# biodatageeks/polars-bio

Measured on AMD Instinct MI355X. Metric: overlap-pairs/sec, higher is better.
Workload: dtype int32; 1 GPU; overlap_100M_5M_24contig; probe_rows=100000000, build_rows=5000000, contigs=24, filter_op=Strict, parallelism=single GPU

## Files before the change

polars-bio_amd/csrc/host_index.hip.h:

```cpp
#pragma once

namespace {

int build_tables(ivj_ctx* ctx, ivj_index* ix);
bool cs_geom(int64_t n, int nc, int want_rows, CsGeom& g);
size_t cs_index_bytes(const CsGeom& g);
void cs_index_carve(ivj_index* ix, char* p);

int ensure_hier(ivj_ctx* ctx, ivj_index* ix) {
    if (ix->hier_built || ix->n <= 0) return IVJ_OK;
    const HierShape h = hier_shape(ix->n);
    const int64_t wgs = (((ix->n + 15) & ~(int64_t)15) + HIER_WG_ROWS - 1) / HIER_WG_ROWS;
    LAUNCH(ctx, "hier_low", k_hier_low, (unsigned)wgs, 256, (const int2*)ix->ep, ix->n, ix->hier, h);
    if (h.nlev >= 3) LAUNCH(ctx, "hier_high", k_hier_high, 1, 256, ix->hier, h, wgs);
    HIP_TRY(hipGetLastError());
    ix->hier_built = true;
    return IVJ_OK;
}

int need_tables(ivj_ctx* ctx, ivj_index* ix) {
    if (!ix->has_tables) return fail(IVJ_ESTATE, "this index was built for merge / cluster only (with_end_order & 2): it has no lookup tables");
    if (ix->tables_built) return IVJ_OK;
    return build_tables(ctx, ix);
}
// ... 91 lines not shown
        int bins_per_row = 2;
        if (ctx->env_joint_bins == 1 || ctx->env_joint_bins == 2) bins_per_row = ctx->env_joint_bins;
        LAUNCH(ctx, "contig_meta", k_contig_meta_joint, grid1d(ix->n_contigs, 256), 256, (const int32_t*)ix->seg,
               (const int32_t*)ix->b_start, (const int32_t*)ix->e_end, ix->n_contigs, bins_per_row, ix->cmeta_j);
        HIP_TRY(hipMemsetAsync(jb_s, 0, (size_t)ix->bins_len * 4, ctx->stream));
        HIP_TRY(hipMemsetAsync(jb_e, 0, (size_t)ix->bins_len * 4, ctx->stream));
        LAUNCH(ctx, "bins_mark", k_bins_mark, grid1d(n, 256), 256, (const int32_t*)ix->b_start, (const int32_t*)ix->b_contig, n,
               ix->n_contigs, (const int4*)ix->cmeta_j, jb_s);
        LAUNCH(ctx, "bins_mark", k_bins_mark, grid1d(n, 256), 256, (const int32_t*)ix->e_end, (const int32_t*)ckeys, n,
               ix->n_contigs, (const int4*)ix->cmeta_j, jb_e);
        lb_max_scan(jb_s, 0);
        lb_max_scan(jb_e, 1);
        LAUNCH(ctx, "joint_records", k_joint_records, grid1d(ix->bins_len, 256), 256, (const uint32_t*)jb_s, (const uint32_t*)jb_e,
               ix->bins_len, (const int32_t*)ix->b_start, (const int32_t*)ix->e_end, (const int4*)ix->cmeta_j, ix->n_contigs, ix->crec);
    }
    ix->has_end_order = true;
    return IVJ_OK;
}

int build_end_table(ivj_ctx* ctx, ivj_index* ix) {
    IVJ_TRY(build_end_order(ctx, ix));
    if (ix->has_end_table || ix->n == 0 || ix->n_contigs <= 0) { ix->has_end_table = true; return IVJ_OK; }
    const int64_t n = ix->n;
    const int64_t lb_tiles = (ix->bins_len + LB_TILE - 1) / LB_TILE;
    const size_t zb = align_up((size_t)lb_tiles * 8) + align_up(16);
    IVJ_TRY(arena_reserve(ctx, zb + 4096));
    char* z = arena_take<char>(ctx, zb);
    HIP_TRY(hipMemsetAsync(z, 0, zb, ctx->stream));
    LAUNCH(ctx, "contig_meta", k_contig_meta, grid1d(ix->n_contigs, 256), 256, (const int32_t*)ix->seg,
           (const int32_t*)ix->e_end, ix->n_contigs, ix->cmeta_e);
    HIP_TRY(hipMemsetAsync(ix->bins_e, 0, (size_t)ix->bins_len * 4, ctx->stream));
    LAUNCH(ctx, "bins_mark", k_bins_mark, grid1d(n, 256), 256, (const int32_t*)ix->e_end, (const int32_t*)ix->b_contig, n,
           ix->n_contigs, (const int4*)ix->cmeta_e, ix->bins_e);
    LAUNCH(ctx, "bins_scan", (k_scan_lb_u32<MaxOp, false>), lb_tiles, OS_THREADS, ix->bins_e, ix->bins_len, 0u,
           (uint32_t*)(z + align_up((size_t)lb_tiles * 8)), (unsigned long long*)z);
    LAUNCH(ctx, "bins_records", k_bins_records, grid1d(ix->bins_len, 256), 256, (const uint32_t*)ix->bins_e, ix->bins_len,
           (const int32_t*)ix->e_end, (const int4*)ix->cmeta_e, ix->n_contigs, ix->brec_e);
    HIP_TRY(hipGetLastError());
    ix->has_end_table = true;
    return IVJ_OK;
}

int build_argmax(ivj_ctx* ctx, ivj_index* ix) {
    if (ix->has_argmax) return IVJ_OK;
    const int64_t n = ix->n;
    if (n == 0) { ix->has_argmax = true; return IVJ_OK; }
    LAUNCH(ctx, "pmax_change", k_pmax_change, grid1d(n, 256), 256, (const int2*)ix->ep, (const int32_t*)ix->b_contig, n, (uint32_t*)ix->pargmax);
    IVJ_TRY((lb_scan_u32<MaxOp, false>(ctx, "argmax_scan", (uint32_t*)ix->pargmax, n, 0u)));
    LAUNCH(ctx, "nearest_records", k_nearest_records, grid1d(n + 1, 256), 256, (const int32_t*)ix->b_start, (const int2*)ix->ep,
           (const int32_t*)ix->b_row, (const int32_t*)ix->b_contig, (const int32_t*)ix->pargmax, n, ix->nrec);
    ix->has_argmax = true;
    return IVJ_OK;
}

int build_lines(ivj_ctx* ctx, ivj_index* ix) {
    if (ix->has_lines) return IVJ_OK;
    if (!ix->has_tables) return fail(IVJ_ESTATE, "this index was built for merge / cluster only (with_end_order & 2): it has no lookup tables");
    const size_t need = (size_t)ix->bins_len * 64;
    if (ix->nline_cap < need) {
        if (ix->nline) { (void)hipFree(ix->nline); ix->nline = nullptr; ix->nline_cap = 0; }
        if (ctx->nl_cache && ctx->nl_cache_cap >= need) {
            ix->nline = reinterpret_cast<int4*>(ctx->nl_cache); ix->nline_cap = ctx->nl_cache_cap;
            ctx->nl_cache = nullptr; ctx->nl_cache_cap = 0;
        } else {
            hipError_t e = hipMalloc((void**)&ix->nline, need);
            if (e != hipSuccess) { ix->nline = nullptr; return fail(IVJ_ENOMEM, std::string("hipMalloc(nearest lines): ") + hipGetErrorString(e)); }
            ix->nline_cap = need;
        }
    }
    IVJ_TRY(need_tables(ctx, ix));
    IVJ_TRY(build_argmax(ctx, ix));
    LAUNCH(ctx, "nearest_lines", k_nearest_lines, grid1d(ix->bins_len * 4, 256), 256, (const uint32_t*)ix->bins, (const int4*)ix->cmeta, ix->n_contigs, (const int4*)ix->nrec,
           (const int32_t*)ix->b_start, (const int2*)ix->ep, (const int32_t*)ix->b_row, ix->bins_len, ix->n, ix->nline);
    HIP_TRY(hipGetLastError());
    ix->has_lines = true;
    return IVJ_OK;
}

int build_rec4(ivj_ctx* ctx, ivj_index* ix) {
    if (ix->has_rec4 || ix->n == 0) return IVJ_OK;
    LAUNCH(ctx, "rec4", k_rec4, grid1d(ix->n, 256), 256, (const int32_t*)ix->b_start, (const int2*)ix->ep, (const int32_t*)ix->b_row, ix->n, ix->rec4);
    HIP_TRY(hipGetLastError());
    ix->has_rec4 = true;
    return IVJ_OK;
}

int build_flat(ivj_ctx* ctx, ivj_index* ix) {
    if (ix->has_flat || ix->n == 0 || ix->n_contigs <= 0) return IVJ_OK;
    IVJ_TRY(need_tables(ctx, ix));
    HIP_TRY(hipMemsetAsync(ix->lot, 0, (size_t)ix->bins_len * 4, ctx->stream));
    LAUNCH(ctx, "lot_mark", k_lot_mark, grid1d(ix->n, 256), 256, (const int2*)ix->ep, (const int32_t*)ix->b_contig, ix->n,
           ix->n_contigs, (const int4*)ix->cmeta, ix->lot);
    IVJ_TRY((lb_scan_u32<MaxOp, false>(ctx, "lot_scan", ix->lot, ix->bins_len, 0u)));
    LAUNCH(ctx, "tab2", k_tab2, grid1d(ix->bins_len, 256), 256, (const uint32_t*)ix->bins, (const uint32_t*)ix->lot, ix->bins_len, ix->tab2);
    HIP_TRY(hipGetLastError());
    IVJ_TRY(build_rec4(ctx, ix));
    ix->has_flat = true;
    return IVJ_OK;
}

int index_sort_v2(ivj_ctx* ctx, ivj_index* ix, const ivj_side* build, const ivj_opts* opts) {
    OsSort S;
    IVJ_TRY(arena_reserve(ctx, os_sort_plan(S, build->n, opts->n_contigs) + 4096));
    os_sort_take(ctx, S);
    IVJ_TRY(os_sort_run(ctx, S, build->contig, build->start, build->end, build->row_id));
    LAUNCH(ctx, "ix_final", k_ix_final, S.tiles, OS_THREADS, (const int4*)S.recA, (const int4*)S.recB, S.n, S.nc, S.cbits, S.meta, S.st_fin, ix->b_start, ix->ep, ix->b_row,
           ix->b_contig, ix->seg, ix->flags);
    HIP_TRY(hipGetLastError());
    return IVJ_OK;
}

bool ix3_wanted(const ivj_ctx* ctx, int64_t n, int nc) {
    if (nc + 1 > V3_MAX_KEYS || n <= 0 || n > (int64_t)V3_CAP * V3_BUCKETS) return false;
    if (ctx->env_ix_v3 >= 0) return ctx->env_ix_v3 != 0;
    if (ctx->ix3_fallback_streak >= 2 && (ctx->ix3_builds_since_fallback & 15) != 15) return false;
    return n >= (128ll << 10) && n <= (7ll << 20);
}
struct V3Plan { int64_t chunk, hist_len, hs_tiles; int nchunks; size_t z_meta, z_st, z_hs, z_tick, zero_bytes; };
V3Plan v3_plan(int64_t n) {
    V3Plan p;
    p.chunk = ((n + 255) / 256 + OS_TILE - 1) / OS_TILE * OS_TILE;
    if (p.chunk < OS_TILE) p.chunk = OS_TILE;
    p.nchunks = (int)((n + p.chunk - 1) / p.chunk);
    p.hist_len = (int64_t)V3_BUCKETS * p.nchunks;
    p.hs_tiles = (p.hist_len + LB_TILE - 1) / LB_TILE;
    p.z_meta = align_up(sizeof(V3Meta)); p.z_st = align_up((size_t)V3_BUCKETS * 8); p.z_hs = align_up((size_t)p.hs_tiles * 8); p.z_tick = align_up(16);
    p.zero_bytes = p.z_meta + p.z_st + p.z_hs + p.z_tick;
    return p;
}
int index_sort_v3(ivj_ctx* ctx, ivj_index* ix, const ivj_side* build, const ivj_opts* opts, bool* done) {
    *done = false;
    const int64_t n = build->n;
    const int nc = opts->n_contigs;
    const int64_t tiles = (n + OS_TILE - 1) / OS_TILE;
    const V3Plan VP = v3_plan(n);
    const int64_t chunk = VP.chunk, hist_len = VP.hist_len, hs_tiles = VP.hs_tiles;
    const int nchunks = VP.nchunks;
    const size_t z_meta = VP.z_meta, z_st = VP.z_st, z_hs = VP.z_hs, zero_bytes = VP.zero_bytes;
    OsSort S;
    const size_t v2_bytes = os_sort_plan(S, n, nc);
    const bool own_z = ix->ix3_z == nullptr;
    IVJ_TRY(arena_reserve(ctx, std::max(v2_bytes, (own_z ? zero_bytes : 0) + align_up((size_t)hist_len * 4) + align_up((size_t)n * 16)) + 4096));
    char* z = own_z ? arena_take<char>(ctx, zero_bytes) : ix->ix3_z;
    uint32_t* hist = arena_take<uint32_t>(ctx, (size_t)hist_len);
    int4* recs = arena_take<int4>(ctx, (size_t)n);
    V3Meta* meta = (V3Meta*)z;
    unsigned long long* st_local = (unsigned long long*)(z + z_meta);
    unsigned long long* st_scan = (unsigned long long*)(z + z_meta + z_st);
    uint32_t* tick_scan = (uint32_t*)(z + z_meta + z_st + z_hs);
    if (own_z) HIP_TRY(hipMemsetAsync(z, 0, zero_bytes, ctx->stream));
    const size_t pass_lds = (size_t)v3_pass_lds().total;
    if (!ctx->ix3_attr_set) {
        HIP_TRY(hipFuncSetAttribute(reinterpret_cast<const void*>(&k_v3_scatter), hipFuncAttributeMaxDynamicSharedMemorySize, (int)pass_lds));
        HIP_TRY(hipFuncSetAttribute(reinterpret_cast<const void*>(&k_v3_local<true>), hipFuncAttributeMaxDynamicSharedMemorySize, 160 * 1024 - 256));
        HIP_TRY(hipFuncSetAttribute(reinterpret_cast<const void*>(&k_v3_local<false>), hipFuncAttributeMaxDynamicSharedMemorySize, 160 * 1024 - 256));
        ctx->ix3_attr_set = true;
    }
    const unsigned sgrid = (unsigned)(tiles < 512 ? tiles : 512);
    LAUNCH(ctx, "ix3_stats", k_v3_stats, sgrid, OS_THREADS, build->start, build->end, build->contig, n, nc, meta);
    LAUNCH(ctx, "ix3_hist", k_v3_hist, nchunks, OS_THREADS, build->contig, build->start, n, nc, meta, (int)chunk, nchunks, hist);
    LAUNCH(ctx, "ix_scan", (k_scan_lb_u32<SumOp, true>), hs_tiles, OS_THREADS, hist, hist_len, 0u, tick_scan, st_scan);
    const int ms_max = ctx->env_ix_merge >= 0 ? std::min(ctx->env_ix_merge, V3_MAX_MERGE) : V3_MAX_MERGE;
    const uint32_t hw_seq = ctx->hw ? ++ctx->hw_seq : 0u;
    LAUNCH(ctx, "ix3_check", k_v3_check, 1, OS_THREADS, (const uint32_t*)hist, nchunks, n, ms_max, meta, ctx->hw_dev, hw_seq);
    if (!ctx->hw) HIP_TRY(hipMemcpyAsync(ctx->h_total + 6, &meta->bad, 8, hipMemcpyDeviceToHost, ctx->stream));
    if (!ctx->ix3_event) HIP_TRY(hipEventCreateWithFlags(&ctx->ix3_event, hipEventDisableTiming));
    HIP_TRY(hipEventRecord(ctx->ix3_event, ctx->stream));
    t_begin(ctx, "ix3_pass");
    hipLaunchKernelGGL(k_v3_scatter, dim3((unsigned)nchunks), dim3(OS_THREADS), pass_lds, ctx->stream, build->contig, build->start, build->end, build->row_id,
                       recs, n, nc, meta, (int)chunk, nchunks, (const uint32_t*)hist);
    t_end(ctx);
    HIP_TRY(hipGetLastError());
    HIP_TRY(wait_event(ctx, ctx->ix3_event));
    uint32_t* hv = reinterpret_cast<uint32_t*>(ctx->h_total + 6);
    if (ctx->hw) {
        const volatile uint32_t* w = reinterpret_cast<volatile uint32_t*>(ctx->hw);
        if (w[2] == hw_seq) { hv[0] = w[0]; hv[1] = w[1]; }
        else {
            ++ctx->hw_misses;
            HIP_TRY(hipMemcpyAsync(ctx->h_total + 6, &meta->bad, 8, hipMemcpyDeviceToHost, ctx->stream));
            HIP_TRY(hipStreamSynchronize(ctx->stream));
        }
    }
    const uint32_t max_bucket = hv[1] & 0xffffffu;
    const int ms = (int)(hv[1] >> 24);
    if (hv[0] != 0u || max_bucket > (uint32_t)V3_CAP) { ++ctx->ix3_fallbacks; ++ctx->ix3_fallback_streak; ctx->ix3_builds_since_fallback = 0; return IVJ_OK; }
    ctx->ix3_fallback_streak = 0;
    const int cap = (int)std::max<uint32_t>(1024u, (max_bucket + 1023u) / 1024u * 1024u);
    const int bin_bits = cap <= 1024 ? 10 : (cap <= 2048 ? 11 : V3_MAX_BIN_BITS);
    const bool stage = ctx->env_ix_stage >= 0 ? ctx->env_ix_stage != 0 : cap <= 2048;
    const size_t local_lds = (size_t)v3_local_lds(cap, 1 << bin_bits, stage).total;
    with_bool(stage, [&](auto STAGE) {
        LAUNCH_LDS(ctx, "ix3_local", k_v3_local<STAGE>, V3_BUCKETS >> ms, OS_THREADS, local_lds, (const int4*)recs, (const uint32_t*)hist, nchunks, n, nc, cap, bin_bits, ms,
                   meta, st_local, ix->b_start, ix->ep, ix->b_row, ix->b_contig, ix->seg, ix->flags);
    });
    HIP_TRY(hipGetLastError());
    *done = true;
    return IVJ_OK;
}

int build_tables(ivj_ctx* ctx, ivj_index* ix) {
    const int nc = ix->n_contigs;
    const int64_t n = ix->n;
    if (n > 0 && nc > 0) {
        const int64_t lb_tiles = (ix->bins_len + LB_TILE - 1) / LB_TILE;
        const size_t zb = align_up((size_t)lb_tiles * 8) + align_up(16);
        IVJ_TRY(arena_reserve(ctx, zb + 4096));
        char* z = arena_take<char>(ctx, zb);
        HIP_TRY(hipMemsetAsync(z, 0, zb, ctx->stream));
        HIP_TRY(hipMemsetAsync(ix->bins, 0, (size_t)ix->bins_len * 4, ctx->stream));
        LAUNCH(ctx, "contig_meta", k_contig_meta, grid1d(nc, 256), 256, (const int32_t*)ix->seg, (const int32_t*)ix->b_start, nc, ix->cmeta);
        LAUNCH(ctx, "bins_mark", k_bins_mark, grid1d(n, 256), 256, (const int32_t*)ix->b_start, (const int32_t*)ix->b_contig, n, nc,
               (const int4*)ix->cmeta, ix->bins);
        LAUNCH(ctx, "bins_scan", (k_scan_lb_u32<MaxOp, false>), lb_tiles, OS_THREADS, ix->bins, ix->bins_len, 0u,
               (uint32_t*)(z + align_up((size_t)lb_tiles * 8)), (unsigned long long*)z);
        LAUNCH(ctx, "bins_records", k_bins_records, grid1d(ix->bins_len, 256), 256, (const uint32_t*)ix->bins, ix->bins_len,
               (const int32_t*)ix->b_start, (const int4*)ix->cmeta, nc, ix->brec);
        HIP_TRY(hipGetLastError());
    }
    ix->tables_built = true;
    return IVJ_OK;
}

int index_build(ivj_ctx* ctx, const ivj_side* build, const ivj_opts* opts, int with_end_order, ivj_index** out) {
    if (2 * build->n + 2 * (int64_t)opts->n_contigs + 64 > 0x7fffffffll)
        return fail(IVJ_EINVAL, "build side too large for the int32 direct-address table (2*rows + 2*contigs must be < 2^31)");
    ivj_index* ix = new ivj_index();
    ix->ctx = ctx; ix->device = ctx->device; ix->n = build->n; ix->n_contigs = opts->n_contigs; ix->table_mode = opts->table_mode;
    const int64_t n = build->n;
    const size_t nn = (size_t)(n > 0 ? n : 1);
    auto cleanup = [&](int code) { ivj_index_free(ix); return code; };
    {
        const size_t col = align_up(nn * 4);
        const size_t nc = (size_t)opts->n_contigs;
        ix->bins_len = 2 * (int64_t)nn + 2 * (int64_t)nc + 16;
        const size_t v3z = (n > 0 && ix3_wanted(ctx, n, opts->n_contigs)) ? v3_plan(n).zero_bytes : 0;
        const size_t small = align_up((nc + 2) * 4) + align_up(16) + 3 * align_up((nc + 1) * 32) + v3z;
        const size_t flat_bytes = align_up((nn + 1) * 16) + 3 * align_up((size_t)ix->bins_len * 4);
        const size_t spl_bytes = align_up((size_t)SL_MAX_BUCKETS * 8) + align_up((size_t)SL_TAB_CONTIGS * 16) +
                                 align_up((size_t)(4 * SL_MAX_BUCKETS + 2 * SL_TAB_CONTIGS) * 4);
        ix->cs_ok = n > 0 && cs_geom(n, opts->n_contigs, opts->slice_rows > 0 ? opts->slice_rows : ctx->sl_env_rows, ix->cs_g);
        const size_t cs_bytes = ix->cs_ok ? cs_index_bytes(ix->cs_g) : 0;
        const size_t hier_bytes = align_up(hier_shape((int64_t)nn).values * 4);
        const size_t need = hier_bytes + cs_bytes + spl_bytes + flat_bytes + 6 * col + align_up(nn * 8) + align_up((nn + 1) * 32) + 2 * align_up((size_t)ix->bins_len * 4) +
                            3 * align_up((size_t)ix->bins_len * 16) + small + 256;
        if (ctx->ix_cache && ctx->ix_cache_cap >= need) {
            ix->slab = ctx->ix_cache; ix->slab_cap = ctx->ix_cache_cap;
            ctx->ix_cache = nullptr; ctx->ix_cache_cap = 0;
        } else {
            hipError_t e = hipMalloc((void**)&ix->slab, need);
            if (e != hipSuccess) return cleanup(fail(IVJ_ENOMEM, std::string("hipMalloc(index): ") + hipGetErrorString(e)));
            ix->slab_cap = need;
        }
        char* p = ix->slab;
        ix->spl = (unsigned long long*)p;
        ix->sl_cm = (int4*)(p + align_up((size_t)SL_MAX_BUCKETS * 8));
        ix->sl_cell = (uint32_t*)((char*)ix->sl_cm + align_up((size_t)SL_TAB_CONTIGS * 16));
        p += spl_bytes;
        ix->ep = (int2*)p; p += align_up(nn * 8);
        ix->b_start = (int32_t*)p; p += col;
        ix->b_row = (int32_t*)p; p += col;
        ix->b_contig = (int32_t*)p; p += col;
        ix->e_end = (int32_t*)p; p += col;
        ix->e_pos = (int32_t*)p; p += col;
        ix->pargmax = (int32_t*)p; p += col;
        ix->nrec = (int4*)p; p += align_up((nn + 1) * 32);
        ix->bins = (uint32_t*)p; p += align_up((size_t)ix->bins_len * 4);
        ix->bins_e = (uint32_t*)p; p += align_up((size_t)ix->bins_len * 4);
        ix->brec = (int4*)p; p += align_up((size_t)ix->bins_len * 16);
        ix->brec_e = (int4*)p; p += align_up((size_t)ix->bins_len * 16);
        ix->crec = (int4*)p; p += align_up((size_t)ix->bins_len * 16);
        ix->rec4 = (int4*)p; p += align_up((nn + 1) * 16);
        {
            ix->lot = (uint32_t*)p; p += align_up((size_t)ix->bins_len * 4);
            ix->tab2 = (uint2*)p; p += 2 * align_up((size_t)ix->bins_len * 4);
        }
        char* small_base = p;
        ix->seg = (int32_t*)p; p += align_up((nc + 2) * 4);
        ix->flags = (int32_t*)p; p += align_up(16);
        ix->cmeta = (int4*)p; p += align_up((nc + 1) * 32);
        ix->cmeta_e = (int4*)p; p += align_up((nc + 1) * 32);
        ix->cmeta_j = (int4*)p; p += align_up((nc + 1) * 32);
        ix->ix3_z = v3z ? p : nullptr; p += v3z;
        if (ix->cs_ok) { cs_index_carve(ix, p); p += cs_bytes; }
        ix->hier = (int32_t*)p;
        hipError_t e = hipMemsetAsync(small_base, 0, small, ctx->stream);
        if (e != hipSuccess) return cleanup(fail(IVJ_EHIP, std::string("hipMemsetAsync(index meta): ") + hipGetErrorString(e)));
    }
    if (n > 0) {
        ix->has_tables = !(with_end_order & 2);
        int r = IVJ_OK;
        bool sorted = false;
        const bool try_v3 = ix3_wanted(ctx, n, opts->n_contigs);
        ++ctx->ix3_builds_since_fallback;
        if (try_v3) { r = index_sort_v3(ctx, ix, build, opts, &sorted); if (r != IVJ_OK) return cleanup(r); }
        if (!sorted) r = index_sort_v2(ctx, ix, build, opts);
        if (r != IVJ_OK) return cleanup(r);
        if (opts->partition_mode == 5) { r = build_flat(ctx, ix); if (r != IVJ_OK) return cleanup(r); }
        if (with_end_order & 1) { r = build_end_order(ctx, ix); if (r != IVJ_OK) return cleanup(r); }
    } else {
        ix->has_end_order = true;
    }
    hipError_t e = hipGetLastError();
    if (e != hipSuccess) return cleanup(fail(IVJ_EHIP, std::string("index build launch: ") + hipGetErrorString(e)));
    ctx->live.push_back(ix);
    *out = ix;
    return IVJ_OK;
}

}
```

polars-bio_amd/csrc/ixsort3.hip.h:

```cpp
#pragma once
#include "onesweep.hip.h"

namespace ivj {

constexpr int V3_BUCKETS = OS_RADIX;
constexpr int V3_ITEMS = 4;
constexpr int V3_CAP = OS_THREADS * V3_ITEMS;
constexpr int V3_MAX_KEYS = 256;
constexpr int V3_MAX_BIN_BITS = 12;

struct V3Meta {
    uint32_t inverted;
    uint32_t pad0;
    uint32_t bad;
    uint32_t max_bucket;
    uint32_t ticket;
    uint32_t wbits;
    uint32_t pad[2];
    unsigned long long M;
    unsigned long long span;
    uint32_t cmax[V3_MAX_KEYS];
    uint32_t cimn[V3_MAX_KEYS];
    uint32_t base[V3_MAX_KEYS];
};
// ... 95 lines not shown
    const int tid = threadIdx.x;
    uint32_t sz[2];
#pragma unroll
    for (int q = 0; q < 2; ++q) {
        const int b = 2 * tid + q;
        const uint32_t a = off[(int64_t)b * nchunks];
        const uint32_t z = b + 1 < V3_BUCKETS ? off[(int64_t)(b + 1) * nchunks] : (uint32_t)n;
        sz[q] = z - a;
    }
    uint32_t mx[V3_MAX_MERGE + 1];
    mx[0] = sz[0] > sz[1] ? sz[0] : sz[1];
    uint32_t sum = sz[0] + sz[1];
    mx[1] = sum;
#pragma unroll
    for (int k = 2; k <= V3_MAX_MERGE; ++k) { sum += __shfl_xor(sum, 1 << (k - 2), kWave); mx[k] = sum; }
#pragma unroll
    for (int k = 0; k <= V3_MAX_MERGE; ++k) {
#pragma unroll
        for (int d = kWave / 2; d > 0; d >>= 1) { const uint32_t o = __shfl_xor(mx[k], d, kWave); mx[k] = o > mx[k] ? o : mx[k]; }
        if ((tid & (kWave - 1)) == 0) wmx[k][tid / kWave] = mx[k];
    }
    __syncthreads();
    if (tid == 0) {
        uint32_t best = 0, best_ms = 0;
#pragma unroll
        for (int k = 0; k <= V3_MAX_MERGE; ++k) {
            uint32_t m = 0;
#pragma unroll
            for (int w = 0; w < OS_WAVES; ++w) m = wmx[k][w] > m ? wmx[k][w] : m;
            if (k == 0 || (k <= ms_max && m <= (uint32_t)V3_CAP)) { best = m; best_ms = (uint32_t)k; }
        }
        meta->max_bucket = best | (best_ms << 24);
        if (hw) { hw_store(hw + 0, 0u); hw_store(hw + 1, best | (best_ms << 24)); hw_store(hw + 2, hw_seq); }
    }
}

struct V3PassLds { OsPassLds P; int tbase, tcmin, total; };
__host__ __device__ inline V3PassLds v3_pass_lds() {
    V3PassLds L;
    L.P = os_pass_lds();
    int o = (L.P.total + 15) & ~15;
    L.tbase = o; o += 4 * V3_MAX_KEYS;
    L.tcmin = o; o += 4 * V3_MAX_KEYS;
    L.total = o;
    return L;
}

__global__ __launch_bounds__(OS_THREADS) void k_v3_scatter(const int32_t* __restrict__ contig, const int32_t* __restrict__ start,
                                                          const int32_t* __restrict__ end, const int32_t* __restrict__ row_id,
                                                          int4* __restrict__ dst, int64_t n, int32_t n_contigs, V3Meta* __restrict__ meta,
                                                          int chunk, int nchunks, const uint32_t* __restrict__ off ) {
    extern __shared__ __attribute__((aligned(16))) unsigned char os_lds[];
    const V3PassLds LL = v3_pass_lds();
    const OsPassLds& L = LL.P;
    int4* l_rec = reinterpret_cast<int4*>(os_lds + L.rec);
    unsigned short* wcnt = reinterpret_cast<unsigned short*>(os_lds + L.wcnt);
    unsigned short* l_d = reinterpret_cast<unsigned short*>(os_lds + L.d);
    uint32_t* base = reinterpret_cast<uint32_t*>(os_lds + L.base);
    uint32_t* lstart = reinterpret_cast<uint32_t*>(os_lds + L.lstart);
    uint32_t* wsum = reinterpret_cast<uint32_t*>(os_lds + L.wsum);
    uint32_t* l_base = reinterpret_cast<uint32_t*>(os_lds + LL.tbase);
    uint32_t* l_cmin = reinterpret_cast<uint32_t*>(os_lds + LL.tcmin);
    if (meta->bad) return;
    const unsigned long long M = meta->M;
    const int tid = threadIdx.x, w = tid / kWave, lane = tid & (kWave - 1);
    v3_load_tables(meta, n_contigs + 1, l_base, l_cmin);
    for (int k = tid; k < OS_RADIX; k += OS_THREADS) base[k] = off[(int64_t)k * nchunks + blockIdx.x];
    for (int k = tid; k < OS_RADIX * OS_WAVES / 2; k += OS_THREADS) reinterpret_cast<uint32_t*>(wcnt)[k] = 0;
    __syncthreads();
    const int64_t cbase = (int64_t)blockIdx.x * chunk;
    const int64_t cend = cbase + chunk < n ? cbase + chunk : n;
    const uint64_t lt = lanemask_lt();
    unsigned short* my = wcnt + w * OS_RADIX;
    const int el0 = w * (OS_ITEMS * kWave) + lane;
    int4 nxt[OS_ITEMS];
    auto load_tile = [&](int64_t tb) {
        const int tn = (int)((cend - tb) < (int64_t)OS_TILE ? (cend - tb) : (int64_t)OS_TILE);
#pragma unroll
        for (int j = 0; j < OS_ITEMS; ++j) {
            const int il = el0 + j * kWave;
            nxt[j] = il < tn ? os_load_record(true, contig, start, end, row_id, nullptr, tb + il, n_contigs) : make_int4(0, 0, 0, 0);
        }
    };
    if (cbase < cend) load_tile(cbase);
    for (int64_t tbase = cbase; tbase < cend; tbase += OS_TILE) {
        const int tile_n = (int)((cend - tbase) < (int64_t)OS_TILE ? (cend - tbase) : (int64_t)OS_TILE);
        int4 r[OS_ITEMS];
        uint32_t d[OS_ITEMS], rank[OS_ITEMS];
#pragma unroll
        for (int j = 0; j < OS_ITEMS; ++j) {
            r[j] = nxt[j];
            d[j] = v3_bucket(l_base[r[j].w] + (flip(r[j].x) - l_cmin[r[j].w]), M);
        }
        if (tbase + OS_TILE < cend) load_tile(tbase + OS_TILE);
#pragma unroll
        for (int j = 0; j < OS_ITEMS; ++j) {
            const bool valid = el0 + j * kWave < tile_n;
            uint64_t peers = __ballot(valid);
#pragma unroll
            for (int b = 0; b < OS_BITS; ++b) {
                const bool bit = (d[j] >> b) & 1u;
                const uint64_t m = __ballot(valid && bit);
                peers &= bit ? m : ~m;
            }
            const uint32_t rk = (uint32_t)__popcll(peers & lt);
            const uint32_t before = valid ? (uint32_t)my[d[j]] : 0u;
            rank[j] = before + rk;
            __builtin_amdgcn_wave_barrier();
            if (valid && rk == 0) my[d[j]] = (unsigned short)(before + (uint32_t)__popcll(peers));
            __builtin_amdgcn_wave_barrier();
        }
        __syncthreads();
        uint32_t x0 = 0, x1 = 0;
        {
            uint32_t* row32 = reinterpret_cast<uint32_t*>(wcnt) + tid;
#pragma unroll
            for (int k = 0; k < OS_WAVES; ++k) {
                const uint32_t v = row32[k * (OS_RADIX / 2)];
                row32[k * (OS_RADIX / 2)] = x0 | (x1 << 16);
                x0 += v & 0xffffu; x1 += v >> 16;
            }
        }
        uint32_t tsum;
        const uint32_t pre = sl_block_exclusive_sum(x0 + x1, wsum, &tsum);
        lstart[2 * tid] = pre;
        lstart[2 * tid + 1] = pre + x0;
        __syncthreads();
#pragma unroll
        for (int j = 0; j < OS_ITEMS; ++j) {
            if (el0 + j * kWave < tile_n) {
                const uint32_t pos = lstart[d[j]] + (uint32_t)my[d[j]] + rank[j];
                l_rec[pos] = r[j];
                l_d[pos] = (unsigned short)d[j];
            }
        }
        __syncthreads();
#pragma unroll
        for (int j = 0; j < OS_ITEMS; ++j) {
            const int il = j * OS_THREADS + tid;
            if (il < tile_n) {
                const uint32_t dd = l_d[il];
                const int4 rr = l_rec[il];
                dst[base[dd] + ((uint32_t)il - lstart[dd])] = rr;
            }
        }
        for (int k = tid; k < OS_RADIX * OS_WAVES / 2; k += OS_THREADS) reinterpret_cast<uint32_t*>(wcnt)[k] = 0;
        __syncthreads();
        base[2 * tid] += x0;
        base[2 * tid + 1] += x1;
        __syncthreads();
    }
}

struct V3LocalLds { int rec, bst, cur, tk, ts, ifin, tbase, tcmin, wsum, total; };
__host__ __device__ inline V3LocalLds v3_local_lds(int cap, int bins, bool stage) {
    V3LocalLds L;
    int o = 0;
    L.rec = o; o += stage ? 16 * cap : 0;
    L.bst = o; o += 4 * (bins + 4);
    L.cur = o; o += 4 * bins;
    L.tk = o; o += 4 * cap;
    L.ts = o; o += 2 * cap;
    L.ifin = o; o += 2 * cap;
    L.tbase = o; o += 4 * V3_MAX_KEYS;
    L.tcmin = o; o += 4 * V3_MAX_KEYS;
    L.wsum = (o + 15) & ~15; o = L.wsum + 8 * OS_WAVES;
    L.total = o;
    return L;
}

template <bool STAGE>
__global__ __launch_bounds__(OS_THREADS, 8) void k_v3_local(const int4* __restrict__ rec, const uint32_t* __restrict__ off, int nchunks, int64_t n,
                                                        int32_t n_contigs, int cap, int bin_bits, int ms, V3Meta* __restrict__ meta, unsigned long long* __restrict__ status64,
                                                        int32_t* __restrict__ b_start, int2* __restrict__ ep, int32_t* __restrict__ b_row,
                                                        int32_t* __restrict__ b_contig, int32_t* __restrict__ seg, int32_t* __restrict__ flags) {
    extern __shared__ __attribute__((aligned(16))) unsigned char os_lds[];
    const int bins = 1 << bin_bits;
    const V3LocalLds L = v3_local_lds(cap, bins, STAGE);
    int4* l_rec = reinterpret_cast<int4*>(os_lds + L.rec);
    uint32_t* bst = reinterpret_cast<uint32_t*>(os_lds + L.bst);
    uint32_t* cur = reinterpret_cast<uint32_t*>(os_lds + L.cur);
    uint32_t* tk = reinterpret_cast<uint32_t*>(os_lds + L.tk);
    unsigned short* ts = reinterpret_cast<unsigned short*>(os_lds + L.ts);
    unsigned short* iF = reinterpret_cast<unsigned short*>(os_lds + L.ifin);
    uint32_t* l_base = reinterpret_cast<uint32_t*>(os_lds + L.tbase);
    uint32_t* l_cmin = reinterpret_cast<uint32_t*>(os_lds + L.tcmin);
    unsigned long long* wmax = reinterpret_cast<unsigned long long*>(os_lds + L.wsum);
    uint32_t* wsum = reinterpret_cast<uint32_t*>(wmax);
    uint32_t* l_pm = tk;
    __shared__ int l_tile;
    __shared__ uint32_t l_lo;
    __shared__ unsigned long long s_carry;
    const int tid = threadIdx.x, w = tid / kWave, lane = tid & (kWave - 1);
    if (tid == 0) {
        const int t = (int)atomicAdd(&meta->ticket, 1u);
        l_tile = t;
        const unsigned long long M = meta->M;
        l_lo = (uint32_t)((((unsigned long long)((unsigned)t << ms) << 32) + M - 1ull) / M);
    }
    v3_load_tables(meta, n_contigs + 1, l_base, l_cmin);
    for (int k = tid; k < bins; k += OS_THREADS) { bst[k] = 0u; cur[k] = 0u; }
    __syncthreads();
    const int tile = l_tile;
    const uint32_t lo = l_lo;
    const int fb0 = tile << ms, fb1 = (tile + 1) << ms;
    const uint32_t b0 = off[(int64_t)fb0 * nchunks];
    const uint32_t b1 = fb1 < V3_BUCKETS ? off[(int64_t)fb1 * nchunks] : (uint32_t)n;
    const int nb = (int)(b1 - b0);
    const int wbits = (int)meta->wbits + ms;
    const int bshift = wbits > bin_bits ? wbits - bin_bits : 0;
    const int4* __restrict__ grec = rec + (int64_t)b0;
    auto row_at = [&](int p) -> int4 { if constexpr (STAGE) return l_rec[p]; else return grec[p]; };

    uint32_t kv[V3_ITEMS];
    unsigned long long cmx = 0ull;
#pragma unroll
    for (int j = 0; j < V3_ITEMS; ++j) {
        const int p = j * OS_THREADS + tid;
        kv[j] = 0u;
        if (p < nb) {
            const int4 r = grec[p];
            if constexpr (STAGE) l_rec[p] = r;
            kv[j] = l_base[r.w] + (flip(r.x) - l_cmin[r.w]) - lo;
            atomicAdd(&bst[kv[j] >> bshift], 1u);
            const unsigned long long c = ((unsigned long long)(uint32_t)r.w << 32) | (unsigned long long)flip(r.y);
            cmx = c > cmx ? c : cmx;
        }
    }
#pragma unroll
    for (int d = kWave / 2; d > 0; d >>= 1) { const unsigned long long o = __shfl_xor(cmx, d, kWave); cmx = o > cmx ? o : cmx; }
    if (lane == 0) wmax[w] = cmx;
    __syncthreads();
    if (tid == 0) {
        unsigned long long tmax = 0;
#pragma unroll
        for (int k = 0; k < OS_WAVES; ++k) tmax = wmax[k] > tmax ? wmax[k] : tmax;
        os_st64(status64 + tile, ((tile == 0 ? 2ull : 1ull) << 62) | tmax);
    }
    {
        const bool own = 4 * tid < bins;
        uint4 c4 = make_uint4(0u, 0u, 0u, 0u);
        if (own) c4 = *reinterpret_cast<const uint4*>(bst + 4 * tid);
        const uint32_t s = c4.x + c4.y + c4.z + c4.w;
        __syncthreads();
        uint32_t tsum;
        uint32_t pre = sl_block_exclusive_sum<uint32_t>(s, wsum, &tsum);
        uint4 o4;
        o4.x = pre; pre += c4.x; o4.y = pre; pre += c4.y; o4.z = pre; pre += c4.z; o4.w = pre;
        if (own) *reinterpret_cast<uint4*>(bst + 4 * tid) = o4;
        if (tid == 0) bst[bins] = (uint32_t)nb;
    }
    __syncthreads();
#pragma unroll
    for (int j = 0; j < V3_ITEMS; ++j) {
        const int p = j * OS_THREADS + tid;
        if (p < nb) {
            const uint32_t bin = kv[j] >> bshift;
            const uint32_t q = bst[bin] + atomicAdd(&cur[bin], 1u);
            tk[q] = kv[j];
            ts[q] = (unsigned short)p;
        }
    }
    __syncthreads();
#pragma unroll
    for (int j = 0; j < V3_ITEMS; ++j) {
        const int p = j * OS_THREADS + tid;
        if (p < nb) {
            const uint32_t bin = kv[j] >> bshift;
            const uint32_t a = bst[bin], z = bst[bin + 1];
            uint32_t r = a;
            for (uint32_t q = a; q < z; ++q) {
                const uint32_t k2 = tk[q];
                const uint32_t s2 = ts[q];
                r += (k2 < kv[j] || (k2 == kv[j] && s2 < (uint32_t)p)) ? 1u : 0u;
            }
            iF[r] = (unsigned short)p;
        }
    }
    __syncthreads();

    unsigned long long comp[V3_ITEMS];
    int32_t cc[V3_ITEMS];
    unsigned long long run = 0;
#pragma unroll
    for (int k = 0; k < V3_ITEMS; ++k) {
        const int q = V3_ITEMS * tid + k;
        unsigned long long c = 0ull;
        cc[k] = 0;
        if (q < nb) {
            const int4 r = row_at(iF[q]);
            c = ((unsigned long long)(uint32_t)r.w << 32) | (unsigned long long)flip(r.y);
            cc[k] = r.w;
        }
        run = c > run ? c : run;
        comp[k] = run;
    }
    int32_t prev_c = -1;
    if (tid > 0 && V3_ITEMS * tid < nb) prev_c = row_at(iF[V3_ITEMS * tid - 1]).w;
    unsigned long long inc = run;
#pragma unroll
    for (int dd = 1; dd < kWave; dd <<= 1) {
        const unsigned long long o = __shfl_up(inc, dd, kWave);
        if (lane >= dd) inc = o > inc ? o : inc;
    }
    if (lane == kWave - 1) wmax[w] = inc;
    if (w == 0) {
        const unsigned long long VAL = (1ull << 62) - 1ull;
        unsigned long long carry = 0;
        for (int t0 = tile - 1; t0 >= 0; t0 -= kWave) {
            const int t = t0 - lane;
            unsigned long long v = 2ull << 62;
            if (t >= 0) {
                v = os_ld64(status64 + t);
                while ((v >> 62) == 0) { __builtin_amdgcn_s_sleep(2); v = os_ld64(status64 + t); }
            }
            const unsigned long long pre_mask = __ballot((v >> 62) == 2ull);
            const int first = pre_mask ? __builtin_ctzll(pre_mask) : kWave;
            unsigned long long x = lane <= first ? (v & VAL) : 0ull;
#pragma unroll
            for (int d = kWave / 2; d > 0; d >>= 1) { const unsigned long long o = __shfl_xor(x, d, kWave); x = o > x ? o : x; }
            carry = x > carry ? x : carry;
            if (pre_mask) break;
        }
        if (lane == 0) s_carry = carry;
    }
    __syncthreads();
    unsigned long long wpre = 0, tmax = 0;
#pragma unroll
    for (int k = 0; k < OS_WAVES; ++k) { const unsigned long long x = wmax[k]; if (k < w) wpre = x > wpre ? x : wpre; tmax = x > tmax ? x : tmax; }
    unsigned long long excl = __shfl_up(inc, 1, kWave);
    if (lane == 0) excl = 0;
    excl = wpre > excl ? wpre : excl;
    if (tid == 0) {
        if (tile > 0) os_st64(status64 + tile, (2ull << 62) | (s_carry > tmax ? s_carry : tmax));
        if (tile == 0) flags[0] = (int32_t)meta->inverted;
    }
    const unsigned long long before = s_carry > excl ? s_carry : excl;
    if (tid == 0) prev_c = b0 == 0u ? -1 : (int32_t)(s_carry >> 32);
#pragma unroll
    for (int k = 0; k < V3_ITEMS; ++k) {
        const int q = V3_ITEMS * tid + k;
        if (q < nb) {
            const unsigned long long pm = before > comp[k] ? before : comp[k];
            l_pm[q] = (uint32_t)pm;
            const int64_t p = (int64_t)b0 + q;
            for (int32_t kk = prev_c + 1; kk <= cc[k]; ++kk) seg[kk] = (int32_t)p;
            prev_c = cc[k];
            if (p == n - 1) for (int32_t kk = cc[k] + 1; kk <= n_contigs + 1; ++kk) seg[kk] = (int32_t)n;
        }
    }
    __syncthreads();
#pragma unroll
    for (int j = 0; j < V3_ITEMS; ++j) {
        const int q = j * OS_THREADS + tid;
        if (q < nb) {
            const int4 r = row_at(iF[q]);
            const int64_t g = (int64_t)b0 + q;
            b_start[g] = r.x;
            ep[g] = make_int2(r.y, unflip(l_pm[q]));
            b_row[g] = r.z;
            b_contig[g] = r.w;
        }
    }
}

}
```

Before: 111.4 billion overlap-pairs/s.

## Replace staged-record local sort with register-held fields and SoA LDS scatter

The default index local-sort kernel no longer stages whole 16-byte records in LDS. It keeps start/end/row/contig in registers, computes each record's rank by counting smaller keys within its bin, scatters the fields into struct-of-arrays LDS, and then writes coalesced outputs. The aim is to cut LDS footprint and the random record gathers of the older path, which remains as an env-selected reread kernel. The risk is the in-bin rank scan, which is quadratic in bin size and adds extra barriers. The look-back scan is also factored into a shared helper.

```diff
diff --git a/polars-bio_amd/csrc/host_index.hip.h b/polars-bio_amd/csrc/host_index.hip.h
--- a/polars-bio_amd/csrc/host_index.hip.h
+++ b/polars-bio_amd/csrc/host_index.hip.h
@@ -267,8 +267,8 @@
     const size_t pass_lds = (size_t)v3_pass_lds().total;
     if (!ctx->ix3_attr_set) {
         HIP_TRY(hipFuncSetAttribute(reinterpret_cast<const void*>(&k_v3_scatter), hipFuncAttributeMaxDynamicSharedMemorySize, (int)pass_lds));
-        HIP_TRY(hipFuncSetAttribute(reinterpret_cast<const void*>(&k_v3_local<true>), hipFuncAttributeMaxDynamicSharedMemorySize, 160 * 1024 - 256));
-        HIP_TRY(hipFuncSetAttribute(reinterpret_cast<const void*>(&k_v3_local<false>), hipFuncAttributeMaxDynamicSharedMemorySize, 160 * 1024 - 256));
+        HIP_TRY(hipFuncSetAttribute(reinterpret_cast<const void*>(&k_v3_local), hipFuncAttributeMaxDynamicSharedMemorySize, 160 * 1024 - 256));
+        HIP_TRY(hipFuncSetAttribute(reinterpret_cast<const void*>(&k_v3_local_reread), hipFuncAttributeMaxDynamicSharedMemorySize, 160 * 1024 - 256));
         ctx->ix3_attr_set = true;
     }
     const unsigned sgrid = (unsigned)(tiles < 512 ? tiles : 512);
@@ -303,12 +303,13 @@
     ctx->ix3_fallback_streak = 0;
     const int cap = (int)std::max<uint32_t>(1024u, (max_bucket + 1023u) / 1024u * 1024u);
     const int bin_bits = cap <= 1024 ? 10 : (cap <= 2048 ? 11 : V3_MAX_BIN_BITS);
-    const bool stage = ctx->env_ix_stage >= 0 ? ctx->env_ix_stage != 0 : cap <= 2048;
-    const size_t local_lds = (size_t)v3_local_lds(cap, 1 << bin_bits, stage).total;
-    with_bool(stage, [&](auto STAGE) {
-        LAUNCH_LDS(ctx, "ix3_local", k_v3_local<STAGE>, V3_BUCKETS >> ms, OS_THREADS, local_lds, (const int4*)recs, (const uint32_t*)hist, nchunks, n, nc, cap, bin_bits, ms,
-                   meta, st_local, ix->b_start, ix->ep, ix->b_row, ix->b_contig, ix->seg, ix->flags);
-    });
+    if (ctx->env_ix_stage == 0) {
+        LAUNCH_LDS(ctx, "ix3_local", k_v3_local_reread, V3_BUCKETS >> ms, OS_THREADS, (size_t)v3_reread_lds(cap, 1 << bin_bits).total, (const int4*)recs, (const uint32_t*)hist,
+                   nchunks, n, nc, cap, bin_bits, ms, meta, st_local, ix->b_start, ix->ep, ix->b_row, ix->b_contig, ix->seg, ix->flags);
+    } else {
+        LAUNCH_LDS(ctx, "ix3_local", k_v3_local, V3_BUCKETS >> ms, OS_THREADS, (size_t)v3_local_lds(cap, 1 << bin_bits).total, (const int4*)recs, (const uint32_t*)hist,
+                   nchunks, n, nc, cap, bin_bits, ms, meta, st_local, ix->b_start, ix->ep, ix->b_row, ix->b_contig, ix->seg, ix->flags);
+    }
     HIP_TRY(hipGetLastError());
     *done = true;
     return IVJ_OK;
diff --git a/polars-bio_amd/csrc/ixsort3.hip.h b/polars-bio_amd/csrc/ixsort3.hip.h
--- a/polars-bio_amd/csrc/ixsort3.hip.h
+++ b/polars-bio_amd/csrc/ixsort3.hip.h
@@ -271,11 +271,236 @@
     }
 }
 
-struct V3LocalLds { int rec, bst, cur, tk, ts, ifin, tbase, tcmin, wsum, total; };
-__host__ __device__ inline V3LocalLds v3_local_lds(int cap, int bins, bool stage) {
+__device__ __forceinline__ unsigned long long v3_look_back(const unsigned long long* __restrict__ status64, int tile, int lane) {
+    const unsigned long long VAL = (1ull << 62) - 1ull;
+    unsigned long long carry = 0;
+    for (int t0 = tile - 1; t0 >= 0; t0 -= kWave) {
+        const int t = t0 - lane;
+        unsigned long long v = 2ull << 62;
+        if (t >= 0) {
+            v = os_ld64(status64 + t);
+            while ((v >> 62) == 0) { __builtin_amdgcn_s_sleep(2); v = os_ld64(status64 + t); }
+        }
+        const unsigned long long pre_mask = __ballot((v >> 62) == 2ull);
+        const int first = pre_mask ? __builtin_ctzll(pre_mask) : kWave;
+        unsigned long long x = lane <= first ? (v & VAL) : 0ull;
+#pragma unroll
+        for (int d = kWave / 2; d > 0; d >>= 1) { const unsigned long long o = __shfl_xor(x, d, kWave); x = o > x ? o : x; }
+        carry = x > carry ? x : carry;
+        if (pre_mask) break;
+    }
+    return carry;
+}
+
+struct V3LocalLds { int bst, tk, ts, sst, sen, srow, sc, tbase, tcmin, wsum, total; };
+__host__ __device__ inline V3LocalLds v3_local_lds(int cap, int bins) {
     V3LocalLds L;
     int o = 0;
-    L.rec = o; o += stage ? 16 * cap : 0;
+    L.bst = o; o += 4 * (bins + 4 > cap ? bins + 4 : cap);
+    L.tk = o; L.ts = o + 4 * cap;
+    L.sst = o; o += 4 * cap;
+    L.sen = o; o += 4 * cap;
+    L.srow = o; o += 4 * cap;
+    L.sc = o; o += cap;
+    L.tbase = o; o += 4 * V3_MAX_KEYS;
+    L.tcmin = o; o += 4 * V3_MAX_KEYS;
+    L.wsum = (o + 15) & ~15; o = L.wsum + 8 * OS_WAVES;
+    L.total = o;
+    return L;
+}
+
+__global__ __launch_bounds__(OS_THREADS, 8) void k_v3_local(const int4* __restrict__ rec, const uint32_t* __restrict__ off, int nchunks, int64_t n,
+                                                        int32_t n_contigs, int cap, int bin_bits, int ms, V3Meta* __restrict__ meta, unsigned long long* __restrict__ status64,
+                                                        int32_t* __restrict__ b_start, int2* __restrict__ ep, int32_t* __restrict__ b_row,
+                                                        int32_t* __restrict__ b_contig, int32_t* __restrict__ seg, int32_t* __restrict__ flags) {
+    extern __shared__ __attribute__((aligned(16))) unsigned char os_lds[];
+    const int bins = 1 << bin_bits;
+    const V3LocalLds L = v3_local_lds(cap, bins);
+    uint32_t* bst = reinterpret_cast<uint32_t*>(os_lds + L.bst);
+    uint32_t* tk = reinterpret_cast<uint32_t*>(os_lds + L.tk);
+    unsigned short* ts = reinterpret_cast<unsigned short*>(os_lds + L.ts);
+    int32_t* s_st = reinterpret_cast<int32_t*>(os_lds + L.sst);
+    int32_t* s_en = reinterpret_cast<int32_t*>(os_lds + L.sen);
+    int32_t* s_row = reinterpret_cast<int32_t*>(os_lds + L.srow);
+    unsigned char* s_c = os_lds + L.sc;
+    uint32_t* l_base = reinterpret_cast<uint32_t*>(os_lds + L.tbase);
+    uint32_t* l_cmin = reinterpret_cast<uint32_t*>(os_lds + L.tcmin);
+    unsigned long long* wmax = reinterpret_cast<unsigned long long*>(os_lds + L.wsum);
+    uint32_t* wsum = reinterpret_cast<uint32_t*>(wmax);
+    uint32_t* l_pm = bst;
+    __shared__ int l_tile;
+    __shared__ uint32_t l_lo;
+    __shared__ unsigned long long s_carry;
+    const int tid = threadIdx.x, w = tid / kWave, lane = tid & (kWave - 1);
+    if (tid == 0) {
+        const int t = (int)atomicAdd(&meta->ticket, 1u);
+        l_tile = t;
+        const unsigned long long M = meta->M;
+        l_lo = (uint32_t)((((unsigned long long)((unsigned)t << ms) << 32) + M - 1ull) / M);
+    }
+    v3_load_tables(meta, n_contigs + 1, l_base, l_cmin);
+    for (int k = tid; k < bins; k += OS_THREADS) bst[k] = 0u;
+    __syncthreads();
+    const int tile = l_tile;
+    const uint32_t lo = l_lo;
+    const int fb0 = tile << ms, fb1 = (tile + 1) << ms;
+    const uint32_t b0 = off[(int64_t)fb0 * nchunks];
+    const uint32_t b1 = fb1 < V3_BUCKETS ? off[(int64_t)fb1 * nchunks] : (uint32_t)n;
+    const int nb = (int)(b1 - b0);
+    const int wbits = (int)meta->wbits + ms;
+    const int bshift = wbits > bin_bits ? wbits - bin_bits : 0;
+    const int4* __restrict__ grec = rec + (int64_t)b0;
+
+    int32_t rs[V3_ITEMS], re[V3_ITEMS], rr[V3_ITEMS];
+    uint32_t kv[V3_ITEMS], rk[V3_ITEMS];
+    unsigned long long cmx = 0ull;
+#pragma unroll
+    for (int j = 0; j < V3_ITEMS; ++j) {
+        const int p = j * OS_THREADS + tid;
+        kv[j] = 0u; rk[j] = 0u;
+        rs[j] = 0; re[j] = 0; rr[j] = 0;
+        if (p < nb) {
+            const int4 r = grec[p];
+            rs[j] = r.x; re[j] = r.y; rr[j] = r.z;
+            rk[j] = (uint32_t)r.w << 16;
+            kv[j] = l_base[r.w] + (flip(r.x) - l_cmin[r.w]) - lo;
+            atomicAdd(&bst[kv[j] >> bshift], 1u);
+            const unsigned long long c = ((unsigned long long)(uint32_t)r.w << 32) | (unsigned long long)flip(r.y);
+            cmx = c > cmx ? c : cmx;
+        }
+    }
+#pragma unroll
+    for (int d = kWave / 2; d > 0; d >>= 1) { const unsigned long long o = __shfl_xor(cmx, d, kWave); cmx = o > cmx ? o : cmx; }
+    if (lane == 0) wmax[w] = cmx;
+    __syncthreads();
+    if (tid == 0) {
+        unsigned long long tmax = 0;
+#pragma unroll
+        for (int k = 0; k < OS_WAVES; ++k) tmax = wmax[k] > tmax ? wmax[k] : tmax;
+        os_st64(status64 + tile, ((tile == 0 ? 2ull : 1ull) << 62) | tmax);
+    }
+    {
+        const bool own = 4 * tid < bins;
+        uint4 c4 = make_uint4(0u, 0u, 0u, 0u);
+        if (own) c4 = *reinterpret_cast<const uint4*>(bst + 4 * tid);
+        const uint32_t s = c4.x + c4.y + c4.z + c4.w;
+        __syncthreads();
+        uint32_t tsum;
+        uint32_t pre = sl_block_exclusive_sum<uint32_t>(s, wsum, &tsum);
+        uint4 o4;
+        o4.x = pre; pre += c4.x; o4.y = pre; pre += c4.y; o4.z = pre; pre += c4.z; o4.w = pre;
+        if (own) *reinterpret_cast<uint4*>(bst + 4 * tid) = o4;
+    }
+    __syncthreads();
+#pragma unroll
+    for (int j = 0; j < V3_ITEMS; ++j) {
+        const int p = j * OS_THREADS + tid;
+        if (p < nb) {
+            const uint32_t q = atomicAdd(&bst[kv[j] >> bshift], 1u);
+            tk[q] = kv[j];
+            ts[q] = (unsigned short)p;
+        }
+    }
+    __syncthreads();
+#pragma unroll
+    for (int j = 0; j < V3_ITEMS; ++j) {
+        const int p = j * OS_THREADS + tid;
+        if (p < nb) {
+            const uint32_t bin = kv[j] >> bshift;
+            const uint32_t a = bin ? bst[bin - 1] : 0u, z = bst[bin];
+            uint32_t x = a;
+            for (uint32_t q = a; q < z; ++q) {
+                const uint32_t k2 = tk[q];
+                const uint32_t s2 = ts[q];
+                x += (k2 < kv[j] || (k2 == kv[j] && s2 < (uint32_t)p)) ? 1u : 0u;
+            }
+            rk[j] |= x;
+        }
+    }
+    __syncthreads();
+#pragma unroll
+    for (int j = 0; j < V3_ITEMS; ++j) {
+        if (j * OS_THREADS + tid < nb) {
+            const uint32_t q = rk[j] & 0xffffu;
+            s_st[q] = rs[j];
+            s_en[q] = re[j];
+            s_row[q] = rr[j];
+            s_c[q] = (unsigned char)(rk[j] >> 16);
+        }
+    }
+    __syncthreads();
+
+    unsigned long long comp[V3_ITEMS];
+    int32_t cc[V3_ITEMS];
+    unsigned long long run = 0;
+#pragma unroll
+    for (int k = 0; k < V3_ITEMS; ++k) {
+        const int q = V3_ITEMS * tid + k;
+        unsigned long long c = 0ull;
+        cc[k] = 0;
+        if (q < nb) {
+            cc[k] = (int32_t)s_c[q];
+            c = ((unsigned long long)(uint32_t)cc[k] << 32) | (unsigned long long)flip(s_en[q]);
+        }
+        run = c > run ? c : run;
+        comp[k] = run;
+    }
+    int32_t prev_c = -1;
+    if (tid > 0 && V3_ITEMS * tid < nb) prev_c = (int32_t)s_c[V3_ITEMS * tid - 1];
+    unsigned long long inc = run;
+#pragma unroll
+    for (int dd = 1; dd < kWave; dd <<= 1) {
+        const unsigned long long o = __shfl_up(inc, dd, kWave);
+        if (lane >= dd) inc = o > inc ? o : inc;
+    }
+    if (lane == kWave - 1) wmax[w] = inc;
+    if (w == 0) {
+        const unsigned long long carry = v3_look_back(status64, tile, lane);
+        if (lane == 0) s_carry = carry;
+    }
+    __syncthreads();
+    unsigned long long wpre = 0, tmax = 0;
+#pragma unroll
+    for (int k = 0; k < OS_WAVES; ++k) { const unsigned long long x = wmax[k]; if (k < w) wpre = x > wpre ? x : wpre; tmax = x > tmax ? x : tmax; }
+    unsigned long long excl = __shfl_up(inc, 1, kWave);
+    if (lane == 0) excl = 0;
+    excl = wpre > excl ? wpre : excl;
+    if (tid == 0) {
+        if (tile > 0) os_st64(status64 + tile, (2ull << 62) | (s_carry > tmax ? s_carry : tmax));
+        if (tile == 0) flags[0] = (int32_t)meta->inverted;
+    }
+    const unsigned long long before = s_carry > excl ? s_carry : excl;
+    if (tid == 0) prev_c = b0 == 0u ? -1 : (int32_t)(s_carry >> 32);
+#pragma unroll
+    for (int k = 0; k < V3_ITEMS; ++k) {
+        const int q = V3_ITEMS * tid + k;
+        if (q < nb) {
+            const unsigned long long pm = before > comp[k] ? before : comp[k];
+            l_pm[q] = (uint32_t)pm;
+            const int64_t p = (int64_t)b0 + q;
+            for (int32_t kk = prev_c + 1; kk <= cc[k]; ++kk) seg[kk] = (int32_t)p;
+            prev_c = cc[k];
+            if (p == n - 1) for (int32_t kk = cc[k] + 1; kk <= n_contigs + 1; ++kk) seg[kk] = (int32_t)n;
+        }
+    }
+    __syncthreads();
+#pragma unroll
+    for (int j = 0; j < V3_ITEMS; ++j) {
+        const int q = j * OS_THREADS + tid;
+        if (q < nb) {
+            const int64_t g = (int64_t)b0 + q;
+            b_start[g] = s_st[q];
+            ep[g] = make_int2(s_en[q], unflip(l_pm[q]));
+            b_row[g] = s_row[q];
+            b_contig[g] = (int32_t)s_c[q];
+        }
+    }
+}
+
+struct V3RereadLds { int bst, cur, tk, ts, ifin, tbase, tcmin, wsum, total; };
+__host__ __device__ inline V3RereadLds v3_reread_lds(int cap, int bins) {
+    V3RereadLds L;
+    int o = 0;
     L.bst = o; o += 4 * (bins + 4);
     L.cur = o; o += 4 * bins;
     L.tk = o; o += 4 * cap;
@@ -288,15 +513,13 @@
     return L;
 }
 
-template <bool STAGE>
-__global__ __launch_bounds__(OS_THREADS, 8) void k_v3_local(const int4* __restrict__ rec, const uint32_t* __restrict__ off, int nchunks, int64_t n,
+__global__ __launch_bounds__(OS_THREADS, 8) void k_v3_local_reread(const int4* __restrict__ rec, const uint32_t* __restrict__ off, int nchunks, int64_t n,
                                                         int32_t n_contigs, int cap, int bin_bits, int ms, V3Meta* __restrict__ meta, unsigned long long* __restrict__ status64,
                                                         int32_t* __restrict__ b_start, int2* __restrict__ ep, int32_t* __restrict__ b_row,
                                                         int32_t* __restrict__ b_contig, int32_t* __restrict__ seg, int32_t* __restrict__ flags) {
     extern __shared__ __attribute__((aligned(16))) unsigned char os_lds[];
     const int bins = 1 << bin_bits;
-    const V3LocalLds L = v3_local_lds(cap, bins, STAGE);
-    int4* l_rec = reinterpret_cast<int4*>(os_lds + L.rec);
+    const V3RereadLds L = v3_reread_lds(cap, bins);
     uint32_t* bst = reinterpret_cast<uint32_t*>(os_lds + L.bst);
     uint32_t* cur = reinterpret_cast<uint32_t*>(os_lds + L.cur);
     uint32_t* tk = reinterpret_cast<uint32_t*>(os_lds + L.tk);
@@ -329,7 +552,7 @@
     const int wbits = (int)meta->wbits + ms;
     const int bshift = wbits > bin_bits ? wbits - bin_bits : 0;
     const int4* __restrict__ grec = rec + (int64_t)b0;
-    auto row_at = [&](int p) -> int4 { if constexpr (STAGE) return l_rec[p]; else return grec[p]; };
+    auto row_at = [&](int p) -> int4 { return grec[p]; };
 
     uint32_t kv[V3_ITEMS];
     unsigned long long cmx = 0ull;
@@ -339,7 +562,6 @@
         kv[j] = 0u;
         if (p < nb) {
             const int4 r = grec[p];
-            if constexpr (STAGE) l_rec[p] = r;
             kv[j] = l_base[r.w] + (flip(r.x) - l_cmin[r.w]) - lo;
             atomicAdd(&bst[kv[j] >> bshift], 1u);
             const unsigned long long c = ((unsigned long long)(uint32_t)r.w << 32) | (unsigned long long)flip(r.y);
@@ -424,23 +646,7 @@
     }
     if (lane == kWave - 1) wmax[w] = inc;
     if (w == 0) {
-        const unsigned long long VAL = (1ull << 62) - 1ull;
-        unsigned long long carry = 0;
-        for (int t0 = tile - 1; t0 >= 0; t0 -= kWave) {
-            const int t = t0 - lane;
-            unsigned long long v = 2ull << 62;
-            if (t >= 0) {
-                v = os_ld64(status64 + t);
-                while ((v >> 62) == 0) { __builtin_amdgcn_s_sleep(2); v = os_ld64(status64 + t); }
-            }
-            const unsigned long long pre_mask = __ballot((v >> 62) == 2ull);
-            const int first = pre_mask ? __builtin_ctzll(pre_mask) : kWave;
-            unsigned long long x = lane <= first ? (v & VAL) : 0ull;
-#pragma unroll
-            for (int d = kWave / 2; d > 0; d >>= 1) { const unsigned long long o = __shfl_xor(x, d, kWave); x = o > x ? o : x; }
-            carry = x > carry ? x : carry;
-            if (pre_mask) break;
-        }
+        const unsigned long long carry = v3_look_back(status64, tile, lane);
         if (lane == 0) s_carry = carry;
     }
     __syncthreads();
```

Result: no change. 112.4 billion overlap-pairs/s (median of 6 runs) (+0.9%).
